# nilsfriess/dune-ddm

Hardware: AMD Instinct MI355X
Metric: preconditioned CG iterations/sec (two-level additive Schwarz), 3D Poisson 10M DoF (higher is better)
Workload: dtype f64

## Files before the change

### dune-ddm_amd/csrc/kernels.hpp

```cpp
#pragma once
#include <hip/hip_runtime.h>
#include <stdint.h>

namespace ddm {

constexpr int WG = 256;
constexpr int SPMV_NNZ = 2048;
constexpr int RED_MAX_BLOCKS = 1024;
constexpr int RED_TRIPS = 4;

__device__ __forceinline__ int xcd_remap(int orig, int nwg)
{
  const int q = nwg >> 3, r = nwg & 7, xcd = orig & 7;
  return (xcd < r ? xcd * (q + 1) : r * (q + 1) + (xcd - r) * q) + (orig >> 3);
}

__device__ __forceinline__ double wave_sum(double v)
{
#pragma unroll
  for (int o = 32; o > 0; o >>= 1) v += __shfl_down(v, o, 64);
  return v;
}

__device__ __forceinline__ double block_sum(double v, double *lds4)
// ... 903 lines not shown
          if (lane == 0) __hip_atomic_store(err, 1u, __ATOMIC_RELAXED, __HIP_MEMORY_SCOPE_SYSTEM);
          break;
        }
      }
      __builtin_amdgcn_fence(__ATOMIC_ACQUIRE, "wavefront");
    }
    DDM_STAMP(t_poll)
#pragma unroll
    for (int u = 0; u < TRSV_UNROLL; ++u) {
      xv[u] = 0.0;
      if (u < H.w) xv[u] = ld_sc1(x + cc[u]);
    }
    double s = upper ? ld_sc1(x + row) : s0;
#pragma unroll
    for (int u = 0; u < TRSV_UNROLL; ++u) s -= vv[u] * xv[u];
    if (H.w > TRSV_UNROLL) {
      const int r = (H.c << 6) + lane;
      const int rr = r < H.m ? r : H.m - 1;
      for (int k = TRSV_UNROLL; k < H.w; ++k)
        s -= valsA[H.ent_off + (int64_t)k * H.m + rr] * ld_sc1(x + colsA[H.ent_off + (int64_t)k * H.m + rr]);
    }
    if (stamp) {
      asm volatile("s_waitcnt vmcnt(0)" ::: "memory");
      DDM_STAMP(t_gather)
    }
    const double out = upper ? s * s0 : s;
    if (act) {
      if (wt) st_sc1(x + row, out);
      else x[row] = out;
    }
    if (H.level_done) {
      asm volatile("s_waitcnt vmcnt(0)" ::: "memory");
      if (lane == 0) {
        unsigned *f = flags + H.flag_base + rank;
        if (wt) __hip_atomic_store(f, epoch, __ATOMIC_RELAXED, __HIP_MEMORY_SCOPE_AGENT);
        else *(volatile unsigned *)f = epoch;
      }
    }
    DDM_STAMP(t_drain)
    n_items += 1;
  }
  if (stamp && lane == 0) {
    stamps[0] = t_tile;
    stamps[1] = t_poll;
    stamps[2] = t_gather;
    stamps[3] = t_drain;
    stamps[4] = n_items;
    stamps[5] = __builtin_amdgcn_s_memtime() - t_begin;
  }
#undef DDM_STAMP
}

__global__ void k_w_permute_in(int64_t n, const int64_t *__restrict__ lpos, const int32_t *__restrict__ rows, const double *__restrict__ d,
                               double *__restrict__ dperm)
{
  for (int64_t i = blockIdx.x * (int64_t)WG + threadIdx.x; i < n; i += (int64_t)gridDim.x * WG) dperm[lpos[i]] = d[rows[lpos[i]]];
}
__global__ void k_w_permute_out(int64_t n, const int64_t *__restrict__ upos, const int32_t *__restrict__ rows, const double *__restrict__ xp,
                                double *__restrict__ x)
{
  for (int64_t i = blockIdx.x * (int64_t)WG + threadIdx.x; i < n; i += (int64_t)gridDim.x * WG) x[rows[upos[i]]] = xp[upos[i]];
}

__global__ void k_perm_gather(int64_t n, int nrhs, const int32_t *__restrict__ perm, const double *__restrict__ src, int64_t ld, double *__restrict__ dst)
{
  const int64_t tot = n * nrhs;
  for (int64_t t = blockIdx.x * (int64_t)WG + threadIdx.x; t < tot; t += (int64_t)gridDim.x * WG) {
    const int64_t i = t / nrhs;
    dst[t] = src[(int64_t)perm[i] * ld + (t - i * nrhs)];
  }
}
__global__ void k_perm_scatter(int64_t n, int nrhs, const int32_t *__restrict__ perm, const double *__restrict__ src, double *__restrict__ dst, int64_t ld)
{
  const int64_t tot = n * nrhs;
  for (int64_t t = blockIdx.x * (int64_t)WG + threadIdx.x; t < tot; t += (int64_t)gridDim.x * WG) {
    const int64_t i = t / nrhs;
    dst[(int64_t)perm[i] * ld + (t - i * nrhs)] = src[t];
  }
}
__global__ void k_perm_scatter_add(int64_t n, int nrhs, const int32_t *__restrict__ perm, const double *__restrict__ src, double *__restrict__ dst, int64_t ld)
{
  const int64_t tot = n * nrhs;
  for (int64_t t = blockIdx.x * (int64_t)WG + threadIdx.x; t < tot; t += (int64_t)gridDim.x * WG) {
    const int64_t i = t / nrhs;
    dst[(int64_t)perm[i] * ld + (t - i * nrhs)] += src[t];
  }
}
__global__ __launch_bounds__(WG) void k_residual_rowmajor(int64_t n, int nrhs, const int64_t *__restrict__ rp, const int32_t *__restrict__ ci, const double *__restrict__ va,
                                                          const double *__restrict__ x, int64_t ldx, const double *__restrict__ d, int64_t ldd, double *__restrict__ r, int64_t ldr)
{
  const int64_t t = (int64_t)blockIdx.x * WG + threadIdx.x;
  const int64_t row = t / nrhs;
  if (row >= n) return;
  const int j = (int)(t - row * nrhs);
  double s = d[row * ldd + j];
  for (int64_t k = rp[row]; k < rp[row + 1]; ++k) s -= va[k] * x[(int64_t)ci[k] * ldx + j];
  r[row * ldr + j] = s;
}
__global__ void k_extend(int64_t n, const int32_t *__restrict__ ext_map, const double *__restrict__ d, double *__restrict__ dov)
{
  for (int64_t i = blockIdx.x * (int64_t)WG + threadIdx.x; i < n; i += (int64_t)gridDim.x * WG) {
    const int32_t m = ext_map[i];
    dov[i] = m >= 0 ? d[m] : 0.0;
  }
}
template <bool ACC, bool SCALE>
__global__ void k_restrict(int64_t n, const int32_t *__restrict__ ext_map, const double *__restrict__ xov,
                           const double *__restrict__ w, double *__restrict__ x)
{
  for (int64_t i = blockIdx.x * (int64_t)WG + threadIdx.x; i < n; i += (int64_t)gridDim.x * WG) {
    const int32_t m = ext_map[i];
    if (m >= 0) {
      const double v = SCALE ? xov[i] * w[i] : xov[i];
      x[m] = ACC ? x[m] + v : v;
    }
  }
}
__global__ void k_scale(int64_t n, const double *__restrict__ w, double *__restrict__ x)
{
  for (int64_t i = blockIdx.x * (int64_t)WG + threadIdx.x; i < n; i += (int64_t)gridDim.x * WG) x[i] *= w[i];
}
__global__ void k_fill(int64_t n, double v, double *__restrict__ x)
{
  for (int64_t i = blockIdx.x * (int64_t)WG + threadIdx.x; i < n; i += (int64_t)gridDim.x * WG) x[i] = v;
}
__global__ void k_axpy(int64_t n, double a, const double *__restrict__ x, double *__restrict__ y)
{
  for (int64_t i = blockIdx.x * (int64_t)WG + threadIdx.x; i < n; i += (int64_t)gridDim.x * WG) y[i] += a * x[i];
}

__global__ void k_axpy_negdev(int64_t n, const double *__restrict__ h, const double *__restrict__ x, double *__restrict__ y)
{
  const double a = h[0];
  for (int64_t i = blockIdx.x * (int64_t)WG + threadIdx.x; i < n; i += (int64_t)gridDim.x * WG) y[i] -= a * x[i];
}
__global__ void k_scal(int64_t n, double a, double *__restrict__ x)
{
  for (int64_t i = blockIdx.x * (int64_t)WG + threadIdx.x; i < n; i += (int64_t)gridDim.x * WG) x[i] *= a;
}

__global__ void k_pack(int64_t n, const int64_t *__restrict__ idx, const double *__restrict__ v, double *__restrict__ buf)
{
  for (int64_t i = blockIdx.x * (int64_t)WG + threadIdx.x; i < n; i += (int64_t)gridDim.x * WG) buf[i] = v[idx[i]];
}
template <bool ADD>
__global__ void k_unpack(int64_t ndst, const int64_t *__restrict__ dst_idx, const int64_t *__restrict__ dst_ptr,
                         const int64_t *__restrict__ src_pos, const double *__restrict__ buf, double *__restrict__ v)
{
  for (int64_t t = blockIdx.x * (int64_t)WG + threadIdx.x; t < ndst; t += (int64_t)gridDim.x * WG) {
    const int64_t i = dst_idx[t];
    double s = ADD ? v[i] : 0.0;
    for (int64_t k = dst_ptr[t]; k < dst_ptr[t + 1]; ++k) s = ADD ? s + buf[src_pos[k]] : buf[src_pos[k]];
    v[i] = s;
  }
}

template <bool MASKED>
__global__ __launch_bounds__(WG) void k_dot_partial(int64_t n, const uint8_t *__restrict__ mask, const double *__restrict__ x,
                                                     const double *__restrict__ y, double *__restrict__ partial)
{
  __shared__ double red[4];
  double s = 0.0;
  const int64_t step = (int64_t)gridDim.x * WG;
  int64_t i = blockIdx.x * (int64_t)WG + threadIdx.x;
  for (; i + (RED_TRIPS - 1) * step < n; i += RED_TRIPS * step) {
    double a[RED_TRIPS], b[RED_TRIPS];
    bool own[RED_TRIPS];
#pragma unroll
    for (int u = 0; u < RED_TRIPS; ++u) a[u] = x[i + u * step], b[u] = y[i + u * step], own[u] = !MASKED || mask[i + u * step];
#pragma unroll
    for (int u = 0; u < RED_TRIPS; ++u)
      if (own[u]) s += a[u] * b[u];
  }
  for (; i < n; i += step)
    if (!MASKED || mask[i]) s += x[i] * y[i];
  s = block_sum(s, red);
  if (threadIdx.x == 0) partial[blockIdx.x] = s;
}
__global__ __launch_bounds__(WG) void k_reduce_final(int nb, const double *__restrict__ partial, double *__restrict__ out)
{
  __shared__ double red[4];
  double s = 0.0;
  for (int i = threadIdx.x; i < nb; i += WG) s += partial[i];
  s = block_sum(s, red);
  if (threadIdx.x == 0) out[0] = s;
}

__global__ void k_cg_lambda(double *scal) { scal[2] = scal[0] / scal[1]; }
__global__ void k_cg_beta(double *scal)
{
  scal[4] = scal[3] / scal[0];
  scal[0] = scal[3];
}
__global__ void k_cg_update(int64_t n, const double *__restrict__ scal, const double *__restrict__ p,
                            const double *__restrict__ q, double *__restrict__ x, double *__restrict__ b)
{
  const double lam = scal[2];
  for (int64_t i = blockIdx.x * (int64_t)WG + threadIdx.x; i < n; i += (int64_t)gridDim.x * WG) {
    x[i] += lam * p[i];
    b[i] -= lam * q[i];
  }
}
template <bool MASKED>
__global__ __launch_bounds__(WG) void k_cg_update_norm(int64_t n, const double *__restrict__ scal, const uint8_t *__restrict__ mask,
                                                        const double *__restrict__ p, const double *__restrict__ q, double *__restrict__ x,
                                                        double *__restrict__ b, double *__restrict__ partial)
{
  __shared__ double red[4];
  const double lam = scal[2];
  double s = 0.0;
  for (int64_t i = blockIdx.x * (int64_t)WG + threadIdx.x; i < n; i += (int64_t)gridDim.x * WG) {
    x[i] += lam * p[i];
    const double bi = b[i] - lam * q[i];
    b[i] = bi;
    if (!MASKED || mask[i]) s += bi * bi;
  }
  s = block_sum(s, red);
  if (threadIdx.x == 0) partial[blockIdx.x] = s;
}
__global__ void k_cg_direction(int64_t n, const double *__restrict__ scal, const double *__restrict__ q, double *__restrict__ p)
{
  const double beta = scal[4];
  for (int64_t i = blockIdx.x * (int64_t)WG + threadIdx.x; i < n; i += (int64_t)gridDim.x * WG) p[i] = beta * p[i] + q[i];
}

constexpr int FCG_SET_MAX = 16;
constexpr int FCG_SG1 = 8;
struct FcgSet {
  int32_t n;
  int32_t buf[FCG_SET_MAX];
};
template <bool MASKED>
__global__ __launch_bounds__(WG) void k_fcg_project(int64_t n, const uint8_t *__restrict__ mask, const double *__restrict__ AD, int64_t stride, FcgSet set,
                                                     int j0, const double *__restrict__ d, double *__restrict__ partial)
{
  __shared__ double red[4];
  double s[FCG_SG1];
  const double *a[FCG_SG1];
#pragma unroll
  for (int j = 0; j < FCG_SG1; ++j) {
    s[j] = 0.0;
    a[j] = AD + (int64_t)set.buf[j < set.n ? j : 0] * stride;
  }
  for (int64_t i = blockIdx.x * (int64_t)WG + threadIdx.x; i < n; i += (int64_t)gridDim.x * WG)
    if (!MASKED || mask[i]) {
      const double di = d[i];
      double ai[FCG_SG1];
#pragma unroll
      for (int j = 0; j < FCG_SG1; ++j) ai[j] = j < set.n ? a[j][i] : 0.0;
#pragma unroll
      for (int j = 0; j < FCG_SG1; ++j) s[j] += ai[j] * di;
    }
#pragma unroll
  for (int j = 0; j < FCG_SG1; ++j) {
    const double t = block_sum(s[j], red);
    if (threadIdx.x == 0 && j < set.n) partial[(int64_t)(j0 + j) * gridDim.x + blockIdx.x] = t;
  }
}
__global__ void k_fcg_coef(FcgSet set, int j0, const double *__restrict__ num, const double *__restrict__ g, double *__restrict__ coef)
{
  const int j = threadIdx.x;
  if (j < set.n) coef[j0 + j] = num[j0 + j] / g[set.buf[j]];
}
__global__ __launch_bounds__(WG) void k_fcg_orth(int64_t n, const double *__restrict__ D, int64_t stride, FcgSet set, int j0, const double *__restrict__ coef,
                                                  double *__restrict__ d)
{
  for (int64_t i = blockIdx.x * (int64_t)WG + threadIdx.x; i < n; i += (int64_t)gridDim.x * WG) {
    double w = d[i];
    for (int j = 0; j < set.n; ++j) w -= coef[j0 + j] * D[(int64_t)set.buf[j] * stride + i];
    d[i] = w;
  }
}
template <bool MASKED>
__global__ __launch_bounds__(WG) void k_fcg_dots(int64_t n, const uint8_t *__restrict__ mask, const double *__restrict__ d, const double *__restrict__ Ad,
                                                  const double *__restrict__ b, double *__restrict__ partial)
{
  __shared__ double red[4];
  double sg = 0.0, sb = 0.0;
  for (int64_t i = blockIdx.x * (int64_t)WG + threadIdx.x; i < n; i += (int64_t)gridDim.x * WG)
    if (!MASKED || mask[i]) {
      const double di = d[i];
      sg += di * Ad[i];
      sb += di * b[i];
    }
  sg = block_sum(sg, red);
  sb = block_sum(sb, red);
  if (threadIdx.x == 0) {
    partial[blockIdx.x] = sg;
    partial[gridDim.x + blockIdx.x] = sb;
  }
}
__global__ void k_fcg_alpha(const double *__restrict__ dots, double *__restrict__ gslot, double *__restrict__ scal)
{
  const double g = dots[0];
  gslot[0] = g;
  scal[2] = g == 0.0 ? __builtin_nan("") : dots[1] / g;
}

static constexpr int COARSE_KMAX = 256;
struct RowChunk {
  int64_t r0, r1;
  int32_t sub, pad;
};
__global__ __launch_bounds__(WG) void k_coarse_restrict_partial(int kmax, int64_t ld, const double *__restrict__ basis,
                                                                 const double *__restrict__ d, const RowChunk *__restrict__ chunks,
                                                                 double *__restrict__ partial , int nchunk)
{
  for (int ch = blockIdx.x; ch < nchunk; ch += gridDim.x) {
  const RowChunk c = chunks[ch];
  const int lane = threadIdx.x & 63, w = threadIdx.x >> 6;
  for (int j = w; j < kmax; j += 4) {
    const double *bj = basis + (int64_t)j * ld;
    double s = 0.0;
    int64_t r = c.r0 + lane;
    for (; r + 7 * 64 < c.r1; r += 8 * 64) {
      double bv[8], dv[8];
#pragma unroll
      for (int u = 0; u < 8; ++u) bv[u] = __builtin_nontemporal_load(bj + r + u * 64);
#pragma unroll
      for (int u = 0; u < 8; ++u) dv[u] = d[r + u * 64];
#pragma unroll
      for (int u = 0; u < 8; ++u) s += bv[u] * dv[u];
    }
    for (; r < c.r1; r += 64) s += bj[r] * d[r];
    s = wave_sum(s);
    if (lane == 0) partial[(int64_t)ch * kmax + j] = s;
  }
  }
}
__global__ __launch_bounds__(WG) void k_coarse_restrict_final(int nsub, int kmax, const int32_t *__restrict__ sub_chunk_ptr,
                                                               const double *__restrict__ partial,
                                                               const int64_t *__restrict__ coarse_index, int64_t K,
                                                               double *__restrict__ d0)
{
  for (int64_t i = threadIdx.x; i < K; i += WG) d0[i] = 0.0;
  __syncthreads();
  for (int t = threadIdx.x; t < nsub * kmax; t += WG) {
    const int s = t / kmax, j = t % kmax;
    const int64_t gi = coarse_index[t];
    if (gi < 0) continue;
    double acc = 0.0;
    for (int c = sub_chunk_ptr[s]; c < sub_chunk_ptr[s + 1]; ++c) acc += partial[(int64_t)c * kmax + j];
    d0[gi] = acc;
  }
}
__global__ __launch_bounds__(WG) void k_dense_mv(int64_t K, const double *__restrict__ M, const double *__restrict__ v,
                                                  double *__restrict__ out)
{
  const int lane = threadIdx.x & 63;
  const int64_t row = blockIdx.x * 4 + (threadIdx.x >> 6);
  if (row >= K) return;
  double s = 0.0;
  for (int64_t c = lane; c < K; c += 64) s += M[row * K + c] * v[c];
  s = wave_sum(s);
  if (lane == 0) out[row] = s;
}
__global__ __launch_bounds__(WG) void k_coarse_prolong(int kmax, int64_t ld, const double *__restrict__ basis,
                                                        const double *__restrict__ x0, const int64_t *__restrict__ coarse_index,
                                                        const RowChunk *__restrict__ chunks, double *__restrict__ xov, int nchunk)
{
  __shared__ double cj[COARSE_KMAX];
  static_assert(COARSE_KMAX <= WG, "one thread per coefficient");
  for (int ch = blockIdx.x; ch < nchunk; ch += gridDim.x) {
  const RowChunk c = chunks[ch];
  __syncthreads();
  if (threadIdx.x < kmax) {
    const int64_t gi = coarse_index[(int64_t)c.sub * kmax + threadIdx.x];
    cj[threadIdx.x] = gi >= 0 ? x0[gi] : 0.0;
  }
  __syncthreads();
  for (int64_t r = c.r0 + threadIdx.x; r < c.r1; r += 2 * WG) {
    const int64_t r2 = r + WG < c.r1 ? r + WG : r;
    double s = 0.0, s2 = 0.0;
    int j = 0;
    for (; j + 4 <= kmax; j += 4) {
      double bv[4], bw[4];
#pragma unroll
      for (int u = 0; u < 4; ++u) bv[u] = __builtin_nontemporal_load(basis + (int64_t)(j + u) * ld + r);
#pragma unroll
      for (int u = 0; u < 4; ++u) bw[u] = __builtin_nontemporal_load(basis + (int64_t)(j + u) * ld + r2);
#pragma unroll
      for (int u = 0; u < 4; ++u) s += cj[j + u] * bv[u];
#pragma unroll
      for (int u = 0; u < 4; ++u) s2 += cj[j + u] * bw[u];
    }
    for (; j < kmax; ++j) {
      s += cj[j] * basis[(int64_t)j * ld + r];
      s2 += cj[j] * basis[(int64_t)j * ld + r2];
    }
    xov[r] = s;
    if (r2 != r) xov[r2] = s2;
  }
  }
}

constexpr int SPREAD_WG = 64;
typedef const __attribute__((address_space(1))) double *uniform_gptr;
__device__ __forceinline__ uniform_gptr uniform_global(const double *p)
{
  const uint64_t v = (uint64_t)p;
  const uint32_t lo = __builtin_amdgcn_readfirstlane((uint32_t)v), hi = __builtin_amdgcn_readfirstlane((uint32_t)(v >> 32));
  return (uniform_gptr)(((uint64_t)hi << 32) | lo);
}
__global__ __launch_bounds__(SPREAD_WG) void k_coarse_restrict_spread(int kmax, int64_t ld, const double *__restrict__ basis,
                                                                       const double *__restrict__ d, const RowChunk *__restrict__ chunks,
                                                                       double *__restrict__ partial , int nchunk)
{
  const int lane = threadIdx.x;
  const int64_t nitem = (int64_t)nchunk * kmax;
  for (int64_t item = blockIdx.x; item < nitem; item += gridDim.x) {
    const int ch = (int)(item / kmax), j = (int)(item % kmax);
    const RowChunk c = chunks[ch];
    const double *bj = basis + (int64_t)j * ld;
    double s = 0.0;
    int64_t r = c.r0 + lane;
    for (; r + 7 * 64 < c.r1; r += 8 * 64) {
      double bv[8], dv[8];
#pragma unroll
      for (int u = 0; u < 8; ++u) bv[u] = __builtin_nontemporal_load(bj + r + u * 64);
#pragma unroll
      for (int u = 0; u < 8; ++u) dv[u] = d[r + u * 64];
#pragma unroll
      for (int u = 0; u < 8; ++u) s += bv[u] * dv[u];
    }
    for (; r < c.r1; r += 64) s += bj[r] * d[r];
    s = wave_sum(s);
    if (lane == 0) partial[item] = s;
  }
}
__global__ __launch_bounds__(SPREAD_WG) void k_coarse_prolong_spread(int kmax, int64_t ld, const double *__restrict__ basis,
                                                                      const double *__restrict__ x0, const int64_t *__restrict__ coarse_index,
                                                                      const RowChunk *__restrict__ chunks, double *__restrict__ xov, int nchunk)
{
  __shared__ double cj[COARSE_KMAX];
  const int lane = threadIdx.x;
  for (int ch = blockIdx.x; ch < nchunk; ch += gridDim.x) {
    const RowChunk c = chunks[ch];
    __syncthreads();
    for (int j = lane; j < kmax; j += SPREAD_WG) {
      const int64_t gi = coarse_index[(int64_t)c.sub * kmax + j];
      cj[j] = gi >= 0 ? x0[gi] : 0.0;
    }
    __syncthreads();
    for (int64_t rb = c.r0; rb < c.r1; rb += 4 * SPREAD_WG) {
      const int nrow = (int)(c.r1 - rb < 4 * SPREAD_WG ? c.r1 - rb : 4 * SPREAD_WG);
      if (lane >= nrow) continue;
      unsigned lo[4];
#pragma unroll
      for (int q = 0; q < 4; ++q) lo[q] = (unsigned)(lane + q * SPREAD_WG < nrow ? lane + q * SPREAD_WG : lane);
      double s[4] = {0.0, 0.0, 0.0, 0.0};
      int j = 0;
#pragma unroll 1
      for (; j + 4 <= kmax; j += 4) {
        double bv[4][4];
#pragma unroll
        for (int u = 0; u < 4; ++u) {
          const uniform_gptr bc = uniform_global(basis + (int64_t)(j + u) * ld + rb);
#pragma unroll
          for (int q = 0; q < 4; ++q) bv[q][u] = __builtin_nontemporal_load(bc + lo[q]);
        }
#pragma unroll
        for (int q = 0; q < 4; ++q)
#pragma unroll
          for (int u = 0; u < 4; ++u) s[q] += cj[j + u] * bv[q][u];
      }
      for (; j < kmax; ++j) {
        const double *bc = basis + (int64_t)j * ld + rb;
#pragma unroll
        for (int q = 0; q < 4; ++q) s[q] += cj[j] * bc[lo[q]];
      }
      xov[rb + lo[0]] = s[0];
#pragma unroll
      for (int q = 1; q < 4; ++q)
        if (lo[q] != (unsigned)lane) xov[rb + lo[q]] = s[q];
    }
  }
}

}
```

### dune-ddm_amd/csrc/preconditioners.hpp

```cpp
#pragma once

static int dot_device(ddm_ctx *ctx, int64_t n, const uint8_t *mask, const double *x, const double *y, double *result_dev)
{
  const int nb = grid_for(n, WG * 4, RED_MAX_BLOCKS);
  if (mask)
    hipLaunchKernelGGL(k_dot_partial<true>, dim3(nb), dim3(WG), 0, ctx->stream, n, mask, x, y, ctx->partial);
  else
    hipLaunchKernelGGL(k_dot_partial<false>, dim3(nb), dim3(WG), 0, ctx->stream, n, mask, x, y, ctx->partial);
  hipLaunchKernelGGL(k_reduce_final, dim3(1), dim3(WG), 0, ctx->stream, nb, ctx->partial, result_dev);
  HIPCHECK(ctx, hipGetLastError());
  DDMCHECK(ctx_allreduce(ctx, result_dev, 1, "scalar product"));
  return DDM_OK;
}

template <class Launch>
static void for_column_groups(int m, Launch &&launch)
{
  for (int c0 = 0; c0 < m;) {
    const int cb = m - c0 >= 8 ? 8 : m - c0 >= 4 ? 4 : m - c0 >= 2 ? 2 : 1;
    launch(c0, cb);
    c0 += cb;
  }
}
#define DDM_MULTI_CB_DISPATCH(KERNEL, MASKED, cb, ...)                                                                 \
// ... 197 lines not shown
                  : ddm_ilu0_create(ctx, A_dir, nblocks, block_ptr, &S->solver));
  DDMCHECK(upload(ctx, ext_map_host, n, S->ext_map));
  if (pou_host) DDMCHECK(upload(ctx, pou_host, n, S->pou));
  if (S->d_ovlp.alloc(n) != hipSuccess || S->x_ovlp.alloc(n) != hipSuccess) return fail(ctx, DDM_EHIP, "alloc");
  *out = S.release();
  return DDM_OK;
}
extern "C" void ddm_schwarz_destroy(ddm_schwarz *S) { delete S; }
extern "C" int64_t ddm_schwarz_num_levels(const ddm_schwarz *S, int upper) { return ddm_ilu0_num_levels(S->solver, upper); }
extern "C" int64_t ddm_schwarz_factor_nnz(const ddm_schwarz *S) { return (S && S->solver) ? S->solver->nnz : 0; }
extern "C" int ddm_schwarz_engine(const ddm_schwarz *S) { return S ? ddm_ilu0_engine(S->solver) : -1; }
extern "C" ddm_ilu0 *ddm_schwarz_local_solver(ddm_schwarz *S) { return S ? S->solver : nullptr; }
extern "C" int ddm_schwarz_status(ddm_ctx *ctx, const ddm_schwarz *S)
{
  if (!S) return fail(ctx, DDM_EINVAL, "ddm_schwarz_status: bad arguments");
  int st = 0;
  DDMCHECK(ddm_ilu0_status(ctx, S->solver, &st));
  if (st) return fail(ctx, DDM_ENUMERIC, "local triangular solve timed out waiting for a dependency (code %d): results are invalid", st);
  return DDM_OK;
}
static int local_status_check(ddm_ctx *ctx, const ddm_schwarz *S)
{
  if (const unsigned e = S ? ilu0_peek_status(S->solver) : 0u)
    return fail(ctx, DDM_ENUMERIC, "an earlier local triangular solve timed out waiting for a dependency (code %u): results since then are invalid", e);
  return DDM_OK;
}
static int schwarz_apply_impl(ddm_ctx *ctx, ddm_schwarz *S, double *x, const double *d, bool acc)
{
  DDMCHECK(local_status_check(ctx, S));
  {
    ScopedTimer t(ctx, "Schwarz/get defect");
    hipLaunchKernelGGL(k_extend, dim3(grid_for(S->n)), dim3(WG), 0, ctx->stream, S->n, S->ext_map, d, S->d_ovlp);
    DDMCHECK(ddm_halo_exchange(ctx, S->copy, S->d_ovlp));
  }
  {
    ScopedTimer t(ctx, "Schwarz/local solve");
    DDMCHECK(ddm_ilu0_solve(ctx, S->solver, S->d_ovlp, S->x_ovlp));
  }
  {
    ScopedTimer t(ctx, "Schwarz/add solution");
    if (S->type == 1 && S->pou)
      hipLaunchKernelGGL(k_scale, dim3(grid_for(S->n)), dim3(WG), 0, ctx->stream, S->n, S->pou, S->x_ovlp);
    DDMCHECK(ddm_halo_exchange(ctx, S->add, S->x_ovlp));
    if (acc)
      hipLaunchKernelGGL((k_restrict<true, false>), dim3(grid_for(S->n)), dim3(WG), 0, ctx->stream, S->n, S->ext_map, S->x_ovlp, (const double *)nullptr, x);
    else
      hipLaunchKernelGGL((k_restrict<false, false>), dim3(grid_for(S->n)), dim3(WG), 0, ctx->stream, S->n, S->ext_map, S->x_ovlp, (const double *)nullptr, x);
    HIPCHECK(ctx, hipGetLastError());
  }
  return DDM_OK;
}
extern "C" int ddm_schwarz_apply(ddm_ctx *ctx, ddm_schwarz *S, double *x, const double *d)
{
  ScopedTimer t(ctx, "Schwarz/apply");
  return schwarz_apply_impl(ctx, S, x, d, false);
}
static int schwarz_multi_scratch(ddm_ctx *ctx, ddm_schwarz *S, int m)
{
  HIPCHECK(ctx, reserve_cols<double>(S->mcols, m, {{S->md_ovlp, S->n}, {S->mx_ovlp, S->n}}));
  return DDM_OK;
}
static int schwarz_apply_multi_impl(ddm_ctx *ctx, ddm_schwarz *S, int m, double *X, const double *D, bool acc)
{
  DDMCHECK(local_status_check(ctx, S));
  DDMCHECK(schwarz_multi_scratch(ctx, S, m));
  {
    ScopedTimer t(ctx, "Schwarz/get defect");
    hipLaunchKernelGGL(k_extend_multi, dim3(grid_for(S->n * m)), dim3(WG), 0, ctx->stream, S->n, m, S->ext_map, D, S->md_ovlp);
    DDMCHECK(halo_exchange_multi(ctx, S->copy, m, S->md_ovlp));
  }
  {
    ScopedTimer t(ctx, "Schwarz/local solve");
    DDMCHECK(ilu0_solve_multi_ld(ctx, S->solver, m, S->md_ovlp, m, S->mx_ovlp, m, S->multi_f32));
  }
  {
    ScopedTimer t(ctx, "Schwarz/add solution");
    if (S->type == 1 && S->pou)
      hipLaunchKernelGGL(k_scale_add_multi, dim3(grid_for(S->n * m)), dim3(WG), 0, ctx->stream, S->n, m, (const double *)S->pou, (const double *)nullptr, S->mx_ovlp);
    DDMCHECK(halo_exchange_multi(ctx, S->add, m, S->mx_ovlp));
    if (acc) hipLaunchKernelGGL(k_restrict_multi<true>, dim3(grid_for(S->n * m)), dim3(WG), 0, ctx->stream, S->n, m, S->ext_map, (const double *)S->mx_ovlp, X);
    else hipLaunchKernelGGL(k_restrict_multi<false>, dim3(grid_for(S->n * m)), dim3(WG), 0, ctx->stream, S->n, m, S->ext_map, (const double *)S->mx_ovlp, X);
    HIPCHECK(ctx, hipGetLastError());
  }
  return DDM_OK;
}
extern "C" int ddm_schwarz_apply_multi(ddm_ctx *ctx, ddm_schwarz *S, int nrhs, double *X, const double *D)
{
  if (!ctx || !S || !X || !D || X == D) return fail(ctx, DDM_EINVAL, "ddm_schwarz_apply_multi: bad arguments");
  DDMCHECK(multi_check(ctx, nrhs, "ddm_schwarz_apply_multi"));
  ScopedTimer t(ctx, "Schwarz/apply");
  return schwarz_apply_multi_impl(ctx, S, nrhs, X, D, false);
}
extern "C" int ddm_schwarz_set_multi_precision(ddm_schwarz *S, int f32)
{
  if (!S) return DDM_EINVAL;
  S->multi_f32 = f32 != 0;
  return DDM_OK;
}
extern "C" int ddm_ilu0_set_status(ddm_ilu0 *F, int status)
{
  if (!F || !F->err) return DDM_EINVAL;
  *(volatile unsigned *)F->err = (unsigned)status;
  return DDM_OK;
}

struct ddm_galerkin {
  int64_t n = 0, n_novlp = 0, nsub = 0, kmax = 0, K = 0, ld = 0;
  dbuf<int32_t> ext_map;
  dbuf<double> basis;
  dbuf<int64_t> coarse_index;
  dbuf<double> a0inv;
  dbuf<RowChunk> chunks;
  dbuf<int32_t> sub_chunk_ptr;
  int nchunk = 0;
  dbuf<double> partial, d0, x0;
  dbuf<double> d_ovlp, x_ovlp;
  ddm_halo *copy = nullptr, *add = nullptr;
  dbuf<double> mpartial, md0, mx0, md_ovlp, mx_ovlp;
  int mcols = 0;
};
static constexpr int64_t COARSE_CHUNK_ROWS = 8192;

extern "C" int ddm_galerkin_create(ddm_ctx *ctx, int64_t n, int64_t n_novlp, const int32_t *ext_map_host, int64_t nsub,
                                   const int64_t *sub_ptr, int64_t kmax, const double *basis_host, const int64_t *coarse_index,
                                   int64_t K, const double *a0inv_host, ddm_halo *ovlp_copy, ddm_halo *ovlp_add,
                                   ddm_galerkin **out)
{
  if (!ctx || !out || !ext_map_host || !sub_ptr || !basis_host || !coarse_index || !a0inv_host)
    return fail(ctx, DDM_EINVAL, "ddm_galerkin_create: bad arguments");
  if (kmax < 1) return fail(ctx, DDM_EINVAL, "Must at least pass one template vector");
  if (kmax > COARSE_KMAX) return fail(ctx, DDM_ENOTIMPL, "more than %d basis vectors per subdomain are not supported", COARSE_KMAX);
  if (sub_ptr[0] != 0 || sub_ptr[nsub] != n) return fail(ctx, DDM_EINVAL, "Template vectors must match size of matrix");
  for (int64_t t = 0; t < nsub * kmax; ++t)
    if (coarse_index[t] >= K) return fail(ctx, DDM_EINVAL, "coarse_index out of range");
  auto G = std::make_unique<ddm_galerkin>();
  G->n = n;
  G->n_novlp = n_novlp;
  G->nsub = nsub;
  G->kmax = kmax;
  G->K = K;
  G->ld = (n + 63) / 64 * 64;
  G->copy = ovlp_copy;
  G->add = ovlp_add;
  std::vector<RowChunk> chunks;
  std::vector<int32_t> scp(nsub + 1, 0);
  for (int64_t s = 0; s < nsub; ++s) {
    for (int64_t r = sub_ptr[s]; r < sub_ptr[s + 1]; r += COARSE_CHUNK_ROWS)
      chunks.push_back(RowChunk{r, std::min(r + COARSE_CHUNK_ROWS, sub_ptr[s + 1]), (int32_t)s, 0});
    scp[s + 1] = (int32_t)chunks.size();
  }
  G->nchunk = (int)chunks.size();
  DDMCHECK(upload(ctx, ext_map_host, n, G->ext_map));
  DDMCHECK(upload(ctx, coarse_index, nsub * kmax, G->coarse_index));
  DDMCHECK(upload(ctx, a0inv_host, K * K, G->a0inv));
  DDMCHECK(upload(ctx, chunks.data(), (int64_t)chunks.size(), G->chunks));
  DDMCHECK(upload(ctx, scp.data(), nsub + 1, G->sub_chunk_ptr));
  if (G->basis.alloc(kmax * G->ld) != hipSuccess || G->partial.alloc((int64_t)G->nchunk * kmax) != hipSuccess ||
      G->d0.alloc(K + 1) != hipSuccess ||
      G->x0.alloc(K) != hipSuccess || G->d_ovlp.alloc(n) != hipSuccess || G->x_ovlp.alloc(n) != hipSuccess)
    return fail(ctx, DDM_EHIP, "galerkin: allocation failed");
  if (hipMemset(G->basis, 0, sizeof(double) * (size_t)(kmax * G->ld)) != hipSuccess) return DDM_EHIP;
  if (hipMemcpy2D(G->basis, sizeof(double) * (size_t)G->ld, basis_host, sizeof(double) * (size_t)n, sizeof(double) * (size_t)n,
                  (size_t)kmax, hipMemcpyHostToDevice) != hipSuccess)
    return fail(ctx, DDM_EHIP, "galerkin: basis upload failed");
  *out = G.release();
  return DDM_OK;
}
extern "C" void ddm_galerkin_destroy(ddm_galerkin *G) { delete G; }
static int coarse_chain(ddm_ctx *ctx, ddm_galerkin *G, const double *dov, int spread_grid = 0)
{
  const unsigned sgrid = (unsigned)spread_grid;
  if (spread_grid > 0)
    hipLaunchKernelGGL(k_coarse_restrict_spread, dim3(sgrid), dim3(SPREAD_WG), 0, ctx->stream, (int)G->kmax, G->ld, G->basis, dov, G->chunks, G->partial, G->nchunk);
  else
    hipLaunchKernelGGL(k_coarse_restrict_partial, dim3(G->nchunk), dim3(WG), 0, ctx->stream, (int)G->kmax, G->ld, G->basis, dov, G->chunks, G->partial, G->nchunk);
  hipLaunchKernelGGL(k_coarse_restrict_final, dim3(1), dim3(WG), 0, ctx->stream, (int)G->nsub, (int)G->kmax, G->sub_chunk_ptr, G->partial, G->coarse_index, G->K, G->d0);
  HIPCHECK(ctx, hipGetLastError());
  DDMCHECK(coarse_allreduce(ctx, G->d0, G->K));
  hipLaunchKernelGGL(k_dense_mv, dim3((unsigned)((G->K + 3) / 4)), dim3(WG), 0, ctx->stream, G->K, G->a0inv, G->d0, G->x0);
  if (spread_grid > 0)
    hipLaunchKernelGGL(k_coarse_prolong_spread, dim3(sgrid), dim3(SPREAD_WG), 0, ctx->stream, (int)G->kmax, G->ld, G->basis, G->x0, G->coarse_index, G->chunks, G->x_ovlp, G->nchunk);
  else
    hipLaunchKernelGGL(k_coarse_prolong, dim3(G->nchunk), dim3(WG), 0, ctx->stream, (int)G->kmax, G->ld, G->basis, G->x0, G->coarse_index, G->chunks, G->x_ovlp, G->nchunk);
  return DDM_OK;
}
static int galerkin_apply_impl(ddm_ctx *ctx, ddm_galerkin *G, double *x, const double *d, bool acc, const double *d_ovlp_ready = nullptr)
{
  ScopedTimer t(ctx, "GalerkinPrec/apply");
  const double *dov = d_ovlp_ready;
  if (!dov) {
    hipLaunchKernelGGL(k_extend, dim3(grid_for(G->n)), dim3(WG), 0, ctx->stream, G->n, G->ext_map, d, G->d_ovlp);
    DDMCHECK(ddm_halo_exchange(ctx, G->copy, G->d_ovlp));
    dov = G->d_ovlp;
  }
  DDMCHECK(coarse_chain(ctx, G, dov));
  DDMCHECK(ddm_halo_exchange(ctx, G->add, G->x_ovlp));
  if (acc)
    hipLaunchKernelGGL((k_restrict<true, false>), dim3(grid_for(G->n)), dim3(WG), 0, ctx->stream, G->n, G->ext_map, G->x_ovlp, (const double *)nullptr, x);
  else
    hipLaunchKernelGGL((k_restrict<false, false>), dim3(grid_for(G->n)), dim3(WG), 0, ctx->stream, G->n, G->ext_map, G->x_ovlp, (const double *)nullptr, x);
  HIPCHECK(ctx, hipGetLastError());
  return DDM_OK;
}
extern "C" int ddm_galerkin_apply(ddm_ctx *ctx, ddm_galerkin *G, double *x, const double *d)
{
  return galerkin_apply_impl(ctx, G, x, d, false);
}
extern "C" int ddm_galerkin_debug_chain(ddm_ctx *ctx, ddm_galerkin *G, const double *d_ovlp, int spread_grid, double *partial_out, double *d0_out,
                                        double *x_ovlp_out, int64_t *npartial)
{
  if (!ctx || !G || !npartial || spread_grid < 0) return fail(ctx, DDM_EINVAL, "ddm_galerkin_debug_chain: bad arguments");
  *npartial = (int64_t)G->nchunk * G->kmax;
  if (!partial_out && !d0_out && !x_ovlp_out) return DDM_OK;
  if (!d_ovlp || !partial_out || !d0_out || !x_ovlp_out) return fail(ctx, DDM_EINVAL, "ddm_galerkin_debug_chain: bad arguments");
  DDMCHECK(coarse_chain(ctx, G, d_ovlp, spread_grid));
  HIPCHECK(ctx, hipMemcpyAsync(partial_out, G->partial, sizeof(double) * (size_t)*npartial, hipMemcpyDeviceToDevice, ctx->stream));
  HIPCHECK(ctx, hipMemcpyAsync(d0_out, G->d0, sizeof(double) * (size_t)G->K, hipMemcpyDeviceToDevice, ctx->stream));
  HIPCHECK(ctx, hipMemcpyAsync(x_ovlp_out, G->x_ovlp, sizeof(double) * (size_t)G->n, hipMemcpyDeviceToDevice, ctx->stream));
  HIPCHECK(ctx, hipStreamSynchronize(ctx->stream));
  return DDM_OK;
}
static int galerkin_multi_scratch(ddm_ctx *ctx, ddm_galerkin *G, int m)
{
  HIPCHECK(ctx, reserve_cols<double>(G->mcols, m, {{G->mpartial, (int64_t)G->nchunk * G->kmax}, {G->md0, G->K}, {G->mx0, G->K}, {G->md_ovlp, G->n}, {G->mx_ovlp, G->n}}));
  return DDM_OK;
}
static int coarse_chain_multi(ddm_ctx *ctx, ddm_galerkin *G, int m, const double *dov)
{
  ScopedTimer t(ctx, "GalerkinPrec/apply");
  hipLaunchKernelGGL(k_coarse_restrict_partial_multi, dim3(G->nchunk), dim3(WG), 0, ctx->stream, (int)G->kmax, G->ld, (const double *)G->basis, m, dov,
                     (const RowChunk *)G->chunks, G->mpartial, G->nchunk);
  hipLaunchKernelGGL(k_coarse_restrict_final_multi, dim3(1), dim3(WG), 0, ctx->stream, (int)G->nsub, (int)G->kmax, m, (const int32_t *)G->sub_chunk_ptr,
                     (const double *)G->mpartial, (const int64_t *)G->coarse_index, G->K, G->md0);
  HIPCHECK(ctx, hipGetLastError());
  DDMCHECK(ctx_allreduce(ctx, G->md0, G->K * m, "coarse defect block"));
  if (G->K > 0)
    hipLaunchKernelGGL(k_dense_mm, dim3((unsigned)((G->K * m + WG - 1) / WG)), dim3(WG), 0, ctx->stream, G->K, m, (const double *)G->a0inv, (const double *)G->md0, G->mx0);
  hipLaunchKernelGGL(k_coarse_prolong_multi, dim3(G->nchunk), dim3(WG), 0, ctx->stream, (int)G->kmax, G->ld, (const double *)G->basis, m, (const double *)G->mx0,
                     (const int64_t *)G->coarse_index, (const RowChunk *)G->chunks, G->mx_ovlp, G->nchunk);
  HIPCHECK(ctx, hipGetLastError());
  return DDM_OK;
}
static int galerkin_apply_multi_impl(ddm_ctx *ctx, ddm_galerkin *G, int m, double *X, const double *D, bool acc, const double *dov_ready = nullptr)
{
  DDMCHECK(galerkin_multi_scratch(ctx, G, m));
  const double *dov = dov_ready;
  if (!dov) {
    hipLaunchKernelGGL(k_extend_multi, dim3(grid_for(G->n * m)), dim3(WG), 0, ctx->stream, G->n, m, G->ext_map, D, G->md_ovlp);
    DDMCHECK(halo_exchange_multi(ctx, G->copy, m, G->md_ovlp));
    dov = G->md_ovlp;
  }
  DDMCHECK(coarse_chain_multi(ctx, G, m, dov));
  DDMCHECK(halo_exchange_multi(ctx, G->add, m, G->mx_ovlp));
  if (acc) hipLaunchKernelGGL(k_restrict_multi<true>, dim3(grid_for(G->n * m)), dim3(WG), 0, ctx->stream, G->n, m, G->ext_map, (const double *)G->mx_ovlp, X);
  else hipLaunchKernelGGL(k_restrict_multi<false>, dim3(grid_for(G->n * m)), dim3(WG), 0, ctx->stream, G->n, m, G->ext_map, (const double *)G->mx_ovlp, X);
  HIPCHECK(ctx, hipGetLastError());
  return DDM_OK;
}
extern "C" int ddm_galerkin_apply_multi(ddm_ctx *ctx, ddm_galerkin *G, int nrhs, double *X, const double *D)
{
  if (!ctx || !G || !X || !D || X == D) return fail(ctx, DDM_EINVAL, "ddm_galerkin_apply_multi: bad arguments");
  DDMCHECK(multi_check(ctx, nrhs, "ddm_galerkin_apply_multi"));
  return galerkin_apply_multi_impl(ctx, G, nrhs, X, D, false);
}

extern "C" int ddm_galerkin_products(ddm_ctx *ctx, const ddm_csr *A_dir, int64_t nleft, const double *left, int64_t nright,
                                     const double *right, int64_t row0, int64_t row1, double *out_host)
{
  if (!A_dir || !left || !right || !out_host || nleft < 1 || nleft > COARSE_KMAX || nright < 1 || row0 < 0 || row1 > A_dir->nrows || row0 > row1)
    return fail(ctx, DDM_EINVAL, "ddm_galerkin_products: bad arguments");
  if (A_dir->host_only) return fail(ctx, DDM_EINVAL, "the matrix was created without device arrays (ddm_csr_create_host)");
  const int64_t n = A_dir->nrows;
  dbuf<double> y, partial, outd;
  dbuf<RowChunk> chunks;
  std::vector<RowChunk> hc;
  for (int64_t r = row0; r < row1; r += COARSE_CHUNK_ROWS) hc.push_back(RowChunk{r, std::min(r + COARSE_CHUNK_ROWS, row1), 0, 0});
  const int nchunk = (int)hc.size();
  HIPCHECK(ctx, y.alloc(n));
  HIPCHECK(ctx, partial.alloc((int64_t)nchunk * nleft));
  HIPCHECK(ctx, outd.alloc(nleft * nright));
  int rc = upload(ctx, hc.data(), (int64_t)hc.size(), chunks);
  std::vector<int32_t> scp = {0, nchunk};
  std::vector<int64_t> cidx(nleft);
  dbuf<int32_t> d_scp;
  dbuf<int64_t> d_cidx;
  if (!rc) rc = upload(ctx, scp.data(), 2, d_scp);
  for (int64_t j = 0; j < nright && !rc; ++j) {
    if (row1 > row0)
      hipLaunchKernelGGL(k_spmm_rowmajor, dim3((unsigned)((row1 - row0 + WG - 1) / WG)), dim3(WG), 0, ctx->stream, row1 - row0, 1, A_dir->rp + row0, A_dir->ci, A_dir->va,
                         right + j * n, (int64_t)1, y + row0, (int64_t)1);
    if (hipGetLastError() != hipSuccess) rc = fail(ctx, DDM_EHIP, "ddm_galerkin_products: kernel launch failed");
    for (int64_t i = 0; i < nleft; ++i) cidx[i] = i;
    if (!d_cidx) rc = upload(ctx, cidx.data(), nleft, d_cidx);
    if (rc) break;
    if (nchunk > 0)
      hipLaunchKernelGGL(k_coarse_restrict_partial, dim3(nchunk), dim3(WG), 0, ctx->stream, (int)nleft, n, left, y, chunks, partial, nchunk);
    hipLaunchKernelGGL(k_coarse_restrict_final, dim3(1), dim3(WG), 0, ctx->stream, 1, (int)nleft, d_scp, partial, d_cidx, nleft, outd + j * nleft);
  }
  if (!rc) rc = ddm_memcpy_d2h(ctx, out_host, outd, sizeof(double) * (size_t)(nleft * nright));
  return rc;
}

constexpr bool OVERLAP_DEFAULT = true;
constexpr int OVERLAP_WAVES_PER_CU = 1;
struct ddm_combined {
  int mode = 0;
  ddm_op *op = nullptr;
  ddm_schwarz *schwarz = nullptr;
  ddm_galerkin *galerkin = nullptr;
  dbuf<double> dnext;
  int64_t n = 0;
  bool fused = false;
  int overlap = 0;
  int side_grid = 0;
  dbuf<double> mdnext, mp, mq;
  dbuf<double> mxw, mbw;
  dbuf<int64_t> mqueue_tab;
  dbuf<double> mrt, mv, my;
  dbuf<double> mz;
  int mcols = 0, mcg_cols = 0, mqueue_cols = 0, mbicg_cols = 0, mbcg_cols = 0;
};
extern "C" int ddm_combined_create(ddm_ctx *ctx, int mode, ddm_op *op, ddm_schwarz *schwarz, ddm_galerkin *galerkin, ddm_combined **out)
{
  if (!ctx || !out || !schwarz) return fail(ctx, DDM_EINVAL, "ERROR: No preconditioners added yet");
  if (mode != 0 && mode != 1) return fail(ctx, DDM_ENOTIMPL, "Unknown apply mode in CombinedPreconditioner, use either additive or multiplicative");
  if (mode == 1 && galerkin && !op) return fail(ctx, DDM_EINVAL, "ERROR: ApplyMode is multiplicative but operator A is not provided. Set with `set_op`");
  auto C = std::make_unique<ddm_combined>();
  C->mode = mode;
  C->op = op;
  C->schwarz = schwarz;
  C->galerkin = galerkin;
  C->n = schwarz->n_novlp;
  if (mode == 0 && galerkin) {
    const char *f = std::getenv("DDM_FUSE_LEVELS");
    const char *e = std::getenv("DDM_OVERLAP_COARSE");
    const char *g = std::getenv("DDM_OVERLAP_GRID");
    C->fused = !(f && f[0] == '0') && galerkin->copy == schwarz->copy && galerkin->add == schwarz->add && galerkin->n == schwarz->n && galerkin->n_novlp == schwarz->n_novlp;
    if (C->fused && (ctx->nranks == 1 || ctx->rccl)) C->overlap = e ? (e[0] == '1' ? 1 : 0) : (OVERLAP_DEFAULT ? 2 : 0);
    C->side_grid = g ? std::max(1, std::atoi(g)) : OVERLAP_WAVES_PER_CU * ctx->num_cu;
  }
  if (C->dnext.alloc(C->n) != hipSuccess) return fail(ctx, DDM_EHIP, "combined: allocation failed");
  *out = C.release();
  return DDM_OK;
}
extern "C" int ddm_combined_status(ddm_ctx *ctx, const ddm_combined *C)
{
  if (!C) return fail(ctx, DDM_EINVAL, "ddm_combined_status: bad arguments");
  return C->schwarz ? ddm_schwarz_status(ctx, C->schwarz) : DDM_OK;
}
extern "C" void ddm_combined_destroy(ddm_combined *C) { delete C; }
static int combined_apply_fused(ddm_ctx *ctx, ddm_combined *C, double *x, const double *d)
{
  ddm_schwarz *S = C->schwarz;
  ddm_galerkin *G = C->galerkin;
  bool pipe_engine = false;
  if (C->overlap != 0) DDMCHECK(ilu0_is_pipe(ctx, S->solver, &pipe_engine));
  const bool two_streams = C->overlap == 1 || (C->overlap == 2 && pipe_engine);
  if (two_streams) DDMCHECK(ctx_side_stream(ctx));
  {
    ScopedTimer t(ctx, "Schwarz/get defect");
    hipLaunchKernelGGL(k_extend, dim3(grid_for(S->n)), dim3(WG), 0, ctx->stream, S->n, S->ext_map, d, S->d_ovlp);
    DDMCHECK(ddm_halo_exchange(ctx, S->copy, S->d_ovlp));
  }
  auto timed_chain = [&](int spread_grid) -> int {
    ScopedTimer t(ctx, "GalerkinPrec/apply");
    return coarse_chain(ctx, G, S->d_ovlp, spread_grid);
  };
  if (two_streams) {
    HIPCHECK(ctx, hipEventRecord(ctx->ev_fork, ctx->stream));
    hipStream_t main = ctx->stream;
    HIPCHECK(ctx, hipStreamWaitEvent(ctx->side, ctx->ev_fork, 0));
    ctx->stream = ctx->side;
    const int rc = timed_chain(C->side_grid);
    const hipError_t e = hipEventRecord(ctx->ev_join, ctx->side);
    ctx->stream = main;
    if (rc) return rc;
    if (e != hipSuccess) return fail(ctx, DDM_EHIP, "hipEventRecord failed: %s", hipGetErrorString(e));
  }
  const double *pou = S->type == 1 ? S->pou : nullptr;
  if (!two_streams) DDMCHECK(timed_chain(0));
  const bool fold = !two_streams || pipe_engine;
  {
    ScopedTimer t(ctx, "Schwarz/local solve");
    DDMCHECK(ilu0_solve_epilogue(ctx, S->solver, S->d_ovlp, S->x_ovlp, fold ? pou : nullptr, fold ? (const double *)G->x_ovlp : nullptr,
                                 two_streams && fold ? ctx->ev_join : nullptr));
  }
  {
    ScopedTimer t(ctx, "Schwarz/add solution");
    if (!fold) {
      if (pou) hipLaunchKernelGGL(k_scale, dim3(grid_for(S->n)), dim3(WG), 0, ctx->stream, S->n, pou, S->x_ovlp);
      HIPCHECK(ctx, hipStreamWaitEvent(ctx->stream, ctx->ev_join, 0));
      hipLaunchKernelGGL(k_axpy, dim3(grid_for(S->n)), dim3(WG), 0, ctx->stream, S->n, 1.0, (const double *)G->x_ovlp, S->x_ovlp);
    }
    DDMCHECK(ddm_halo_exchange(ctx, S->add, S->x_ovlp));
    hipLaunchKernelGGL((k_restrict<false, false>), dim3(grid_for(S->n)), dim3(WG), 0, ctx->stream, S->n, S->ext_map, S->x_ovlp, (const double *)nullptr, x);
    HIPCHECK(ctx, hipGetLastError());
  }
  return DDM_OK;
}

extern "C" int ddm_combined_apply(ddm_ctx *ctx, ddm_combined *C, double *x, const double *d)
{
  ScopedTimer t(ctx, "CombinedPreconditioner/apply");
  DDMCHECK(local_status_check(ctx, C->schwarz));
  if (C->mode == 0 && C->galerkin && C->fused) return combined_apply_fused(ctx, C, x, d);
  DDMCHECK(schwarz_apply_impl(ctx, C->schwarz, x, d, false));
  if (!C->galerkin) return DDM_OK;
  if (C->mode == 0) {
    static const bool no_share = std::getenv("DDM_NO_SHARED_DEFECT") != nullptr;
    const bool share = !no_share && C->galerkin->copy == C->schwarz->copy && C->galerkin->n == C->schwarz->n && C->galerkin->n_novlp == C->schwarz->n_novlp;
    return galerkin_apply_impl(ctx, C->galerkin, x, d, true, share ? C->schwarz->d_ovlp : nullptr);
  }
  HIPCHECK(ctx, hipMemcpyAsync(C->dnext, d, sizeof(double) * (size_t)C->n, hipMemcpyDeviceToDevice, ctx->stream));
  DDMCHECK(ddm_op_applyscaleadd(ctx, C->op, -1.0, x, C->dnext));
  return galerkin_apply_impl(ctx, C->galerkin, x, C->dnext, true);
}
static int combined_apply_multi_impl(ddm_ctx *ctx, ddm_combined *C, int m, double *X, const double *D)
{
  ScopedTimer t(ctx, "CombinedPreconditioner/apply");
  ddm_schwarz *S = C->schwarz;
  ddm_galerkin *G = C->galerkin;
  DDMCHECK(local_status_check(ctx, S));
  if (C->mode == 0 && G && C->fused) {
    DDMCHECK(schwarz_multi_scratch(ctx, S, m));
    DDMCHECK(galerkin_multi_scratch(ctx, G, m));
    {
      ScopedTimer t2(ctx, "Schwarz/get defect");
      hipLaunchKernelGGL(k_extend_multi, dim3(grid_for(S->n * m)), dim3(WG), 0, ctx->stream, S->n, m, S->ext_map, D, S->md_ovlp);
      DDMCHECK(halo_exchange_multi(ctx, S->copy, m, S->md_ovlp));
    }
    DDMCHECK(coarse_chain_multi(ctx, G, m, S->md_ovlp));
    {
      ScopedTimer t2(ctx, "Schwarz/local solve");
      DDMCHECK(ilu0_solve_multi_ld(ctx, S->solver, m, S->md_ovlp, m, S->mx_ovlp, m, S->multi_f32));
    }
    {
      ScopedTimer t2(ctx, "Schwarz/add solution");
      const double *pou = S->type == 1 ? S->pou : nullptr;
      hipLaunchKernelGGL(k_scale_add_multi, dim3(grid_for(S->n * m)), dim3(WG), 0, ctx->stream, S->n, m, pou, (const double *)G->mx_ovlp, S->mx_ovlp);
      DDMCHECK(halo_exchange_multi(ctx, S->add, m, S->mx_ovlp));
      hipLaunchKernelGGL(k_restrict_multi<false>, dim3(grid_for(S->n * m)), dim3(WG), 0, ctx->stream, S->n, m, S->ext_map, (const double *)S->mx_ovlp, X);
      HIPCHECK(ctx, hipGetLastError());
    }
    return DDM_OK;
  }
  DDMCHECK(schwarz_apply_multi_impl(ctx, S, m, X, D, false));
  if (!G) return DDM_OK;
  if (C->mode == 0) {
    const bool share = G->copy == S->copy && G->n == S->n && G->n_novlp == S->n_novlp;
    return galerkin_apply_multi_impl(ctx, G, m, X, D, true, share ? S->md_ovlp : nullptr);
  }
  HIPCHECK(ctx, reserve_cols(C->mcols, m, C->mdnext, C->n));
  HIPCHECK(ctx, hipMemcpyAsync(C->mdnext, D, sizeof(double) * (size_t)(C->n * m), hipMemcpyDeviceToDevice, ctx->stream));
  DDMCHECK(op_applyscaleadd_multi(ctx, C->op, m, -1.0, X, C->mdnext));
  return galerkin_apply_multi_impl(ctx, G, m, X, C->mdnext, true);
}
extern "C" int ddm_combined_apply_multi(ddm_ctx *ctx, ddm_combined *C, int nrhs, double *X, const double *D)
{
  if (!ctx || !C || !X || !D || X == D) return fail(ctx, DDM_EINVAL, "ddm_combined_apply_multi: bad arguments");
  DDMCHECK(multi_check(ctx, nrhs, "ddm_combined_apply_multi"));
  return combined_apply_multi_impl(ctx, C, nrhs, X, D);
}
```

Baseline: 229.2.

## Reuse d across basis vector groups in coarse restrict, vectorize prolong, size side grid

```diff
diff --git a/dune-ddm_amd/csrc/kernels.hpp b/dune-ddm_amd/csrc/kernels.hpp
--- a/dune-ddm_amd/csrc/kernels.hpp
+++ b/dune-ddm_amd/csrc/kernels.hpp
@@ -1229,30 +1229,68 @@
   int64_t r0, r1;
   int32_t sub, pad;
 };
+typedef const __attribute__((address_space(1))) double *uniform_gptr;
+__device__ __forceinline__ uniform_gptr uniform_global(const double *p)
+{
+  const uint64_t v = (uint64_t)p;
+  const uint32_t lo = __builtin_amdgcn_readfirstlane((uint32_t)v), hi = __builtin_amdgcn_readfirstlane((uint32_t)(v >> 32));
+  return (uniform_gptr)(((uint64_t)hi << 32) | lo);
+}
+constexpr int COARSE_JG = 10, COARSE_JG_FULL = 5;
+template <int JG>
+__device__ __forceinline__ void restrict_group(const double *__restrict__ b0, int64_t vstride, const RowChunk c, int lane,
+                                               const double *__restrict__ d, double *__restrict__ out, int ostride)
+{
+  double s[JG];
+#pragma unroll
+  for (int jj = 0; jj < JG; ++jj) s[jj] = 0.0;
+  int64_t rb = c.r0;
+  for (; rb + 8 * 64 <= c.r1; rb += 8 * 64) {
+    const uniform_gptr dc = uniform_global(d + rb);
+    double dv[8];
+#pragma unroll
+    for (int u = 0; u < 8; ++u) dv[u] = __builtin_nontemporal_load(dc + (unsigned)(lane + u * 64));
+#pragma unroll
+    for (int p = 0; p < JG; p += 2) {
+      const int nv = p + 1 < JG ? 2 : 1;
+      double bv[2][8];
+#pragma unroll
+      for (int v = 0; v < nv; ++v) {
+        const uniform_gptr bc = uniform_global(b0 + (int64_t)(p + v) * vstride + rb);
+#pragma unroll
+        for (int u = 0; u < 8; ++u) bv[v][u] = __builtin_nontemporal_load(bc + (unsigned)(lane + u * 64));
+      }
+#pragma unroll
+      for (int v = 0; v < nv; ++v)
+#pragma unroll
+        for (int u = 0; u < 8; ++u) s[p + v] += bv[v][u] * dv[u];
+      __builtin_amdgcn_sched_barrier(0);
+    }
+  }
+  for (; rb < c.r1; rb += 64) {
+    if (rb + lane >= c.r1) continue;
+    const double dr = __builtin_nontemporal_load(d + rb + lane);
+    const uniform_gptr bc = uniform_global(b0 + rb);
+#pragma unroll
+    for (int jj = 0; jj < JG; ++jj) s[jj] += bc[(int64_t)jj * vstride + lane] * dr;
+  }
+#pragma unroll
+  for (int jj = 0; jj < JG; ++jj) {
+    const double t = wave_sum(s[jj]);
+    if (lane == 0) out[(int64_t)jj * ostride] = t;
+  }
+}
 __global__ __launch_bounds__(WG) void k_coarse_restrict_partial(int kmax, int64_t ld, const double *__restrict__ basis,
                                                                  const double *__restrict__ d, const RowChunk *__restrict__ chunks,
                                                                  double *__restrict__ partial , int nchunk)
 {
+  const int lane = threadIdx.x & 63, w = threadIdx.x >> 6;
   for (int ch = blockIdx.x; ch < nchunk; ch += gridDim.x) {
-  const RowChunk c = chunks[ch];
-  const int lane = threadIdx.x & 63, w = threadIdx.x >> 6;
-  for (int j = w; j < kmax; j += 4) {
-    const double *bj = basis + (int64_t)j * ld;
-    double s = 0.0;
-    int64_t r = c.r0 + lane;
-    for (; r + 7 * 64 < c.r1; r += 8 * 64) {
-      double bv[8], dv[8];
-#pragma unroll
-      for (int u = 0; u < 8; ++u) bv[u] = __builtin_nontemporal_load(bj + r + u * 64);
-#pragma unroll
-      for (int u = 0; u < 8; ++u) dv[u] = d[r + u * 64];
-#pragma unroll
-      for (int u = 0; u < 8; ++u) s += bv[u] * dv[u];
-    }
-    for (; r < c.r1; r += 64) s += bj[r] * d[r];
-    s = wave_sum(s);
-    if (lane == 0) partial[(int64_t)ch * kmax + j] = s;
-  }
+    const RowChunk c = chunks[ch];
+    int j = w;
+    for (; j + 4 * (COARSE_JG_FULL - 1) < kmax; j += 4 * COARSE_JG_FULL)
+      restrict_group<COARSE_JG_FULL>(basis + (int64_t)j * ld, 4 * ld, c, lane, d, partial + (int64_t)ch * kmax + j, 4);
+    for (; j < kmax; j += 4) restrict_group<1>(basis + (int64_t)j * ld, 4 * ld, c, lane, d, partial + (int64_t)ch * kmax + j, 4);
   }
 }
 __global__ __launch_bounds__(WG) void k_coarse_restrict_final(int nsub, int kmax, const int32_t *__restrict__ sub_chunk_ptr,
@@ -1322,39 +1360,26 @@
 }
 
 constexpr int SPREAD_WG = 64;
-typedef const __attribute__((address_space(1))) double *uniform_gptr;
-__device__ __forceinline__ uniform_gptr uniform_global(const double *p)
-{
-  const uint64_t v = (uint64_t)p;
-  const uint32_t lo = __builtin_amdgcn_readfirstlane((uint32_t)v), hi = __builtin_amdgcn_readfirstlane((uint32_t)(v >> 32));
-  return (uniform_gptr)(((uint64_t)hi << 32) | lo);
-}
 __global__ __launch_bounds__(SPREAD_WG) void k_coarse_restrict_spread(int kmax, int64_t ld, const double *__restrict__ basis,
                                                                        const double *__restrict__ d, const RowChunk *__restrict__ chunks,
                                                                        double *__restrict__ partial , int nchunk)
 {
   const int lane = threadIdx.x;
-  const int64_t nitem = (int64_t)nchunk * kmax;
+  const int nfull = kmax / COARSE_JG, ngroup = nfull + (kmax % COARSE_JG != 0);
+  const int64_t nitem = (int64_t)nchunk * ngroup;
   for (int64_t item = blockIdx.x; item < nitem; item += gridDim.x) {
-    const int ch = (int)(item / kmax), j = (int)(item % kmax);
+    const int ch = (int)(item / ngroup), g = (int)(item % ngroup);
     const RowChunk c = chunks[ch];
-    const double *bj = basis + (int64_t)j * ld;
-    double s = 0.0;
-    int64_t r = c.r0 + lane;
-    for (; r + 7 * 64 < c.r1; r += 8 * 64) {
-      double bv[8], dv[8];
-#pragma unroll
-      for (int u = 0; u < 8; ++u) bv[u] = __builtin_nontemporal_load(bj + r + u * 64);
-#pragma unroll
-      for (int u = 0; u < 8; ++u) dv[u] = d[r + u * 64];
-#pragma unroll
-      for (int u = 0; u < 8; ++u) s += bv[u] * dv[u];
-    }
-    for (; r < c.r1; r += 64) s += bj[r] * d[r];
-    s = wave_sum(s);
-    if (lane == 0) partial[item] = s;
-  }
-}
+    const double *b0 = basis + (int64_t)g * COARSE_JG * ld;
+    double *out = partial + (int64_t)ch * kmax + g * COARSE_JG;
+    if (g < nfull)
+      restrict_group<COARSE_JG>(b0, ld, c, lane, d, out, 1);
+    else
+      for (int j = 0; j < kmax - nfull * COARSE_JG; ++j) restrict_group<1>(b0 + (int64_t)j * ld, ld, c, lane, d, out + j, 1);
+  }
+}
+typedef double double2_t __attribute__((ext_vector_type(2)));
+typedef const __attribute__((address_space(1))) double2_t *uniform_gptr2;
 __global__ __launch_bounds__(SPREAD_WG) void k_coarse_prolong_spread(int kmax, int64_t ld, const double *__restrict__ basis,
                                                                       const double *__restrict__ x0, const int64_t *__restrict__ coarse_index,
                                                                       const RowChunk *__restrict__ chunks, double *__restrict__ xov, int nchunk)
@@ -1369,39 +1394,56 @@
       cj[j] = gi >= 0 ? x0[gi] : 0.0;
     }
     __syncthreads();
-    for (int64_t rb = c.r0; rb < c.r1; rb += 4 * SPREAD_WG) {
-      const int nrow = (int)(c.r1 - rb < 4 * SPREAD_WG ? c.r1 - rb : 4 * SPREAD_WG);
-      if (lane >= nrow) continue;
-      unsigned lo[4];
-#pragma unroll
-      for (int q = 0; q < 4; ++q) lo[q] = (unsigned)(lane + q * SPREAD_WG < nrow ? lane + q * SPREAD_WG : lane);
-      double s[4] = {0.0, 0.0, 0.0, 0.0};
+    const int64_t ra = c.r0 + (c.r0 & 1), re = ra + ((c.r1 - ra) & ~(int64_t)1);
+    {
+      const int64_t rs = lane == 0 && ra != c.r0 ? c.r0 : lane == 1 && re < c.r1 ? re : -1;
+      if (rs >= 0) {
+        double s = 0.0;
+        for (int j = 0; j < kmax; ++j) s += cj[j] * basis[(int64_t)j * ld + rs];
+        xov[rs] = s;
+      }
+    }
+    for (int64_t rb = ra; rb < re; rb += 4 * SPREAD_WG) {
+      const int npair = (int)(re - rb < 4 * SPREAD_WG ? re - rb : 4 * SPREAD_WG) / 2;
+      if (lane >= npair) continue;
+      unsigned lo[2];
+#pragma unroll
+      for (int q = 0; q < 2; ++q) lo[q] = (unsigned)(lane + q * SPREAD_WG < npair ? lane + q * SPREAD_WG : lane);
+      double2_t s[2] = {{0.0, 0.0}, {0.0, 0.0}};
       int j = 0;
 #pragma unroll 1
       for (; j + 4 <= kmax; j += 4) {
-        double bv[4][4];
+        double2_t bv[2][4];
 #pragma unroll
         for (int u = 0; u < 4; ++u) {
-          const uniform_gptr bc = uniform_global(basis + (int64_t)(j + u) * ld + rb);
-#pragma unroll
-          for (int q = 0; q < 4; ++q) bv[q][u] = __builtin_nontemporal_load(bc + lo[q]);
+          const uniform_gptr2 bc = (uniform_gptr2)uniform_global(basis + (int64_t)(j + u) * ld + rb);
+#pragma unroll
+          for (int q = 0; q < 2; ++q) bv[q][u] = __builtin_nontemporal_load(bc + lo[q]);
         }
 #pragma unroll
-        for (int q = 0; q < 4; ++q)
-#pragma unroll
-          for (int u = 0; u < 4; ++u) s[q] += cj[j + u] * bv[q][u];
+        for (int q = 0; q < 2; ++q)
+#pragma unroll
+          for (int u = 0; u < 4; ++u) {
+            const double cu = cj[j + u];
+            s[q].x += cu * bv[q][u].x;
+            s[q].y += cu * bv[q][u].y;
+          }
       }
       for (; j < kmax; ++j) {
-        const double *bc = basis + (int64_t)j * ld + rb;
-#pragma unroll
-        for (int q = 0; q < 4; ++q) s[q] += cj[j] * bc[lo[q]];
-      }
-      xov[rb + lo[0]] = s[0];
-#pragma unroll
-      for (int q = 1; q < 4; ++q)
-        if (lo[q] != (unsigned)lane) xov[rb + lo[q]] = s[q];
-    }
-  }
-}
-
-}
+        const double2_t *bc = (const double2_t *)(basis + (int64_t)j * ld + rb);
+        const double cu = cj[j];
+#pragma unroll
+        for (int q = 0; q < 2; ++q) {
+          const double2_t b = bc[lo[q]];
+          s[q].x += cu * b.x;
+          s[q].y += cu * b.y;
+        }
+      }
+      double2_t *xo = (double2_t *)(xov + rb);
+      xo[lo[0]] = s[0];
+      if (lo[1] != (unsigned)lane) xo[lo[1]] = s[1];
+    }
+  }
+}
+
+}
diff --git a/dune-ddm_amd/csrc/preconditioners.hpp b/dune-ddm_amd/csrc/preconditioners.hpp
--- a/dune-ddm_amd/csrc/preconditioners.hpp
+++ b/dune-ddm_amd/csrc/preconditioners.hpp
@@ -523,7 +523,13 @@
 }
 
 constexpr bool OVERLAP_DEFAULT = true;
-constexpr int OVERLAP_WAVES_PER_CU = 1;
+constexpr int OVERLAP_WAVES_PER_16_CU = 7, OVERLAP_KMAX_MEASURED = 20;
+static int overlap_default_grid(int num_cu, int64_t kmax)
+{
+  const int64_t k = std::max<int64_t>(kmax, OVERLAP_KMAX_MEASURED);
+  const int64_t g = (OVERLAP_WAVES_PER_16_CU * num_cu * k + 16 * OVERLAP_KMAX_MEASURED - 1) / (16 * OVERLAP_KMAX_MEASURED);
+  return (int)std::max<int64_t>(1, std::min<int64_t>(g, num_cu));
+}
 struct ddm_combined {
   int mode = 0;
   ddm_op *op = nullptr;
@@ -558,7 +564,7 @@
     const char *g = std::getenv("DDM_OVERLAP_GRID");
     C->fused = !(f && f[0] == '0') && galerkin->copy == schwarz->copy && galerkin->add == schwarz->add && galerkin->n == schwarz->n && galerkin->n_novlp == schwarz->n_novlp;
     if (C->fused && (ctx->nranks == 1 || ctx->rccl)) C->overlap = e ? (e[0] == '1' ? 1 : 0) : (OVERLAP_DEFAULT ? 2 : 0);
-    C->side_grid = g ? std::max(1, std::atoi(g)) : OVERLAP_WAVES_PER_CU * ctx->num_cu;
+    C->side_grid = g ? std::max(1, std::atoi(g)) : overlap_default_grid(ctx->num_cu, galerkin->kmax);
   }
   if (C->dnext.alloc(C->n) != hipSuccess) return fail(ctx, DDM_EHIP, "combined: allocation failed");
   *out = C.release();
```

Result: no change. 232.1, median of 6 (+1.3%).
